# argmaxinc/WhisperKit

Hardware: NVIDIA H100
Metric: RTFx (audio-sec/s) whisper-large-v3 greedy (higher is better)
Workload: dtype bf16

## Files before the change

### whisperkit_b200/csrc/attention_wgmma.cu

```cuda
#include <stdio.h>
#include <stdlib.h>

#include "common.cuh"
#include "kernels.h"
#include "wgmma.cuh"

namespace wk {

static constexpr int kFaThreads = 384;
static constexpr int kFaBM = 128;
static constexpr int kFaBN = 128;
static constexpr int kFaD = 64;
static constexpr int kFaTile = kFaBN * kFaD * 2;
static constexpr int kFaStages = 4;
static constexpr int kFaSmem = kFaTile  + 2 * kFaStages * kFaTile  + 1024  + 256 ;

struct FaParams {
    int T, H, dm, n_kv_tiles;
    float scale_log2e;
};

__device__ __forceinline__ float fa_ex2(float x) {
    float y;
    asm("ex2.approx.ftz.f32 %0, %1;" : "=f"(y) : "f"(x));
    return y;
}

template <typename T>
__global__ void __launch_bounds__(kFaThreads, 1)
encoder_attention_wgmma_kernel(const __grid_constant__ CUtensorMap tm_qkv, T* __restrict__ out, const FaParams p) {
    extern __shared__ __align__(1024) uint8_t smem_raw[];
    uint8_t* smem = reinterpret_cast<uint8_t*>((reinterpret_cast<uintptr_t>(smem_raw) + 1023) & ~uintptr_t(1023));
    uint8_t* sQ = smem;
    uint8_t* sK = sQ + kFaTile;
    uint8_t* sV = sK + kFaStages * kFaTile;
    uint64_t* bars = reinterpret_cast<uint64_t*>(sV + kFaStages * kFaTile);
    uint64_t* q_full = bars;
    uint64_t* k_full = bars + 1;
    uint64_t* k_empty = k_full + kFaStages;
    uint64_t* v_full = k_empty + kFaStages;
    uint64_t* v_empty = v_full + kFaStages;

    const int warp = threadIdx.x >> 5, lane = threadIdx.x & 31;
    const int bh = blockIdx.y;
    const int b = bh / p.H, h = bh % p.H;
    const int q0 = blockIdx.x * kFaBM;
    const int n = p.n_kv_tiles;

    if (warp == 0 && lane == 0) {
        tma_prefetch_desc(&tm_qkv);
        mbar_init(q_full, 1);
        for (int i = 0; i < kFaStages; ++i) {
            mbar_init(&k_full[i], 1); mbar_init(&k_empty[i], 8);
            mbar_init(&v_full[i], 1); mbar_init(&v_empty[i], 8);
        }
        fence_barrier_init();
    }
    __syncthreads();

    if (warp < 4) {
        asm volatile("setmaxnreg.dec.sync.aligned.u32 40;");
        if (warp == 0 && lane == 0) {
            mbar_expect_tx(q_full, kFaTile);
            tma_load_3d(sQ, &tm_qkv, q_full, h * kFaD, q0, b);
            for (int j = 0; j < n; ++j) {
                const int st = j % kFaStages;
                const uint32_t ph = (j / kFaStages) & 1;
                mbar_wait_bounded(&k_empty[st], ph ^ 1);
                mbar_expect_tx(&k_full[st], kFaTile);
                tma_load_3d(sK + st * kFaTile, &tm_qkv, &k_full[st], p.dm + h * kFaD, j * kFaBN, b);
                mbar_wait_bounded(&v_empty[st], ph ^ 1);
                mbar_expect_tx(&v_full[st], kFaTile);
                tma_load_3d(sV + st * kFaTile, &tm_qkv, &v_full[st], 2 * p.dm + h * kFaD, j * kFaBN, b);
            }
        }
        return;
    }

    asm volatile("setmaxnreg.inc.sync.aligned.u32 232;");
    const int cw = (warp >> 2) - 1;
    const int c_lo = 2 * (lane & 3);
    const float c = p.scale_log2e;
    const uint64_t qd = wgmma_desc_sw128(smem_u32(sQ + cw * 64 * 128));
    float o[32];
#pragma unroll
    for (int i = 0; i < 32; ++i) o[i] = 0.f;
    float m_run[2] = {-INFINITY, -INFINITY}, l_run[2] = {0.f, 0.f};

    mbar_wait_bounded(q_full, 0);
    for (int j = 0; j < n; ++j) {
        const int st = j % kFaStages;
        const uint32_t ph = (j / kFaStages) & 1;
        float s[64];
        mbar_wait_bounded(&k_full[st], ph);
        const uint64_t kd = wgmma_desc_sw128(smem_u32(sK + st * kFaTile));
        wgmma_fence();
#pragma unroll
        for (int k = 0; k < kFaD / 16; ++k) Wgmma<T, 128>::ss(s, qd + (uint64_t)(2 * k), kd + (uint64_t)(2 * k), k > 0 ? 1u : 0u);
        wgmma_commit();
        wgmma_wait<0>();
        __syncwarp();
        if (lane == 0) mbar_arrive(&k_empty[st]);

        const int valid = p.T - j * kFaBN;
        if (valid < kFaBN) {
#pragma unroll
            for (int jj = 0; jj < 16; ++jj)
#pragma unroll
                for (int e = 0; e < 4; ++e)
                    if (8 * jj + c_lo + (e & 1) >= valid) s[4 * jj + e] = -INFINITY;
        }
        uint32_t pa[8][4];
#pragma unroll
        for (int hf = 0; hf < 2; ++hf) {
            float mx = m_run[hf];
#pragma unroll
            for (int jj = 0; jj < 16; ++jj) mx = fmaxf(mx, fmaxf(s[4 * jj + 2 * hf], s[4 * jj + 2 * hf + 1]));
            mx = fmaxf(mx, __shfl_xor_sync(0xffffffffu, mx, 1));
            mx = fmaxf(mx, __shfl_xor_sync(0xffffffffu, mx, 2));
            const float corr = fa_ex2((m_run[hf] - mx) * c);
            m_run[hf] = mx;
            const float nmc = -mx * c;
            float sum = 0.f;
#pragma unroll
            for (int jj = 0; jj < 16; ++jj) {
                const float e0 = fa_ex2(fmaf(s[4 * jj + 2 * hf], c, nmc));
                const float e1 = fa_ex2(fmaf(s[4 * jj + 2 * hf + 1], c, nmc));
                sum += e0 + e1;
                pa[jj >> 1][(jj & 1) * 2 + hf] = T16<T>::pack2(e0, e1);
            }
            l_run[hf] = l_run[hf] * corr + sum;
#pragma unroll
            for (int jj = 0; jj < 8; ++jj) { o[4 * jj + 2 * hf] *= corr; o[4 * jj + 2 * hf + 1] *= corr; }
        }

        mbar_wait_bounded(&v_full[st], ph);
        const uint32_t vs = smem_u32(sV + st * kFaTile);
        wgmma_fence();
#pragma unroll
        for (int kk = 0; kk < kFaBN / 16; ++kk) Wgmma<T, 64>::rs_bt(o, pa[kk], wgmma_desc_sw128(vs + kk * 2048), 1u);
        wgmma_commit();
        wgmma_wait<0>();
        __syncwarp();
        if (lane == 0) mbar_arrive(&v_empty[st]);
    }

#pragma unroll
    for (int hf = 0; hf < 2; ++hf) {
        float l = l_run[hf];
        l += __shfl_xor_sync(0xffffffffu, l, 1);
        l += __shfl_xor_sync(0xffffffffu, l, 2);
        const float inv = 1.f / l;
        const int q = q0 + cw * 64 + (warp & 3) * 16 + (lane >> 2) + 8 * hf;
        if (q >= p.T) continue;
        T* dst = out + ((long long)b * p.T + q) * p.dm + h * kFaD + c_lo;
#pragma unroll
        for (int jj = 0; jj < 8; ++jj)
            *reinterpret_cast<uint32_t*>(dst + 8 * jj) = T16<T>::pack2(o[4 * jj + 2 * hf] * inv, o[4 * jj + 2 * hf + 1] * inv);
    }
}

typedef CUresult (*PFN_encodeTiled)(CUtensorMap*, CUtensorMapDataType, cuuint32_t, void*, const cuuint64_t*, const cuuint64_t*,
                                      const cuuint32_t*, const cuuint32_t*, CUtensorMapInterleave, CUtensorMapSwizzle,
                                      CUtensorMapL2promotion, CUtensorMapFloatOOBfill);

wk_status encoder_attention_wgmma(const void* qkv, void* out, int B, int T, int n_heads, int dtype, cudaStream_t stream) {
    static PFN_encodeTiled enc = nullptr;
    if (!enc) {
        void* fp = nullptr;
        cudaDriverEntryPointQueryResult q;
        if (cudaGetDriverEntryPoint("cuTensorMapEncodeTiled", &fp, cudaEnableDefault, &q) != cudaSuccess || q != cudaDriverEntryPointSuccess) {
            set_error("cuTensorMapEncodeTiled entry point unavailable");
            return WK_ERR_CUDA;
        }
        enc = reinterpret_cast<PFN_encodeTiled>(fp);
    }
    const int dm = n_heads * 64;
    CUtensorMap tm;
    cuuint64_t gdim[3] = {(cuuint64_t)3 * dm, (cuuint64_t)T, (cuuint64_t)B};
    cuuint64_t gstr[2] = {(cuuint64_t)3 * dm * 2, (cuuint64_t)T * 3 * dm * 2};
    cuuint32_t box[3] = {64, 128, 1};
    cuuint32_t es[3] = {1, 1, 1};
    CUresult r = enc(&tm, dtype == WK_DTYPE_F16 ? CU_TENSOR_MAP_DATA_TYPE_FLOAT16 : CU_TENSOR_MAP_DATA_TYPE_BFLOAT16, 3,
                     const_cast<void*>(qkv), gdim, gstr, box, es, CU_TENSOR_MAP_INTERLEAVE_NONE, CU_TENSOR_MAP_SWIZZLE_128B,
                     CU_TENSOR_MAP_L2_PROMOTION_L2_256B, CU_TENSOR_MAP_FLOAT_OOB_FILL_NONE);
    if (r != CUDA_SUCCESS) { set_error("attention tensor map encode failed: %d", (int)r); return WK_ERR_CUDA; }
    FaParams p;
    p.T = T; p.H = n_heads; p.dm = dm;
    p.n_kv_tiles = (T + kFaBN - 1) / kFaBN;
    p.scale_log2e = 0.125f * 1.4426950408889634f;
    dim3 grid((T + kFaBM - 1) / kFaBM, B * n_heads);
    cudaError_t e = cudaSuccess;
    if (dtype == WK_DTYPE_F16) {
        static bool set = false;
        if (!set) { e = cudaFuncSetAttribute(encoder_attention_wgmma_kernel<__half>, cudaFuncAttributeMaxDynamicSharedMemorySize, kFaSmem); set = e == cudaSuccess; }
        if (e == cudaSuccess) encoder_attention_wgmma_kernel<__half><<<grid, kFaThreads, kFaSmem, stream>>>(tm, (__half*)out, p);
    } else {
        static bool set = false;
        if (!set) { e = cudaFuncSetAttribute(encoder_attention_wgmma_kernel<__nv_bfloat16>, cudaFuncAttributeMaxDynamicSharedMemorySize, kFaSmem); set = e == cudaSuccess; }
        if (e == cudaSuccess) encoder_attention_wgmma_kernel<__nv_bfloat16><<<grid, kFaThreads, kFaSmem, stream>>>(tm, (__nv_bfloat16*)out, p);
    }
    if (e != cudaSuccess) { set_error("cudaFuncSetAttribute(fa): %s", cudaGetErrorString(e)); return WK_ERR_CUDA; }
    count_launch();
    e = cudaGetLastError();
    if (e != cudaSuccess) { set_error("encoder_attention_wgmma launch: %s", cudaGetErrorString(e)); return WK_ERR_CUDA; }
    return WK_OK;
}

}
```

Measured before the change: 923.4.

## Make encoder flash attention persistent with three consumer warpgroups and QK/PV overlap

Converts the encoder attention kernel into a persistent kernel sized to the SM count. Each CTA now walks work items with a double-buffered Q slot, and the KV stage ring runs across items. Consumer warpgroups go from 2 to 3, so each item covers a 192-row query block. Inside an item, the QK wgmma for the next tile is issued before the PV wgmma of the current tile, which overlaps softmax with tensor-core work. The cost is a lower register budget per thread (160), extra Q smem, and more complex barrier logic. A second TMA load for Q rows beyond T depends on OOB fill.

```diff
diff --git a/whisperkit_b200/csrc/attention_wgmma.cu b/whisperkit_b200/csrc/attention_wgmma.cu
--- a/whisperkit_b200/csrc/attention_wgmma.cu
+++ b/whisperkit_b200/csrc/attention_wgmma.cu
@@ -7,16 +7,18 @@
 
 namespace wk {
 
-static constexpr int kFaThreads = 384;
-static constexpr int kFaBM = 128;
+static constexpr int kFaThreads = 512;
+static constexpr int kFaConsumers = 3;
+static constexpr int kFaBM = 64 * kFaConsumers;
 static constexpr int kFaBN = 128;
 static constexpr int kFaD = 64;
 static constexpr int kFaTile = kFaBN * kFaD * 2;
 static constexpr int kFaStages = 4;
-static constexpr int kFaSmem = kFaTile  + 2 * kFaStages * kFaTile  + 1024  + 256 ;
+static constexpr int kFaQSlot = 2 * kFaTile;
+static constexpr int kFaSmem = 2 * kFaQSlot  + 2 * kFaStages * kFaTile  + 1024  + 256 ;
 
 struct FaParams {
-    int T, H, dm, n_kv_tiles;
+    int T, H, dm, n_kv_tiles, n_q_blocks, n_items;
     float scale_log2e;
 };
 
@@ -24,6 +26,14 @@
     float y;
     asm("ex2.approx.ftz.f32 %0, %1;" : "=f"(y) : "f"(x));
     return y;
+}
+
+__device__ __forceinline__ void fa_wait(uint64_t* bar, uint32_t parity) {
+    if (mbar_try_wait(bar, parity)) return;
+    const unsigned long long t0 = globaltimer_ns();
+    unsigned int spins = 0;
+    while (!mbar_try_wait(bar, parity))
+        if ((++spins & 0xfffu) == 0 && globaltimer_ns() - t0 > kSpinLimitNs) __trap();
 }
 
 template <typename T>
@@ -32,76 +42,81 @@
     extern __shared__ __align__(1024) uint8_t smem_raw[];
     uint8_t* smem = reinterpret_cast<uint8_t*>((reinterpret_cast<uintptr_t>(smem_raw) + 1023) & ~uintptr_t(1023));
     uint8_t* sQ = smem;
-    uint8_t* sK = sQ + kFaTile;
+    uint8_t* sK = sQ + 2 * kFaQSlot;
     uint8_t* sV = sK + kFaStages * kFaTile;
     uint64_t* bars = reinterpret_cast<uint64_t*>(sV + kFaStages * kFaTile);
     uint64_t* q_full = bars;
-    uint64_t* k_full = bars + 1;
+    uint64_t* q_empty = bars + 2;
+    uint64_t* k_full = bars + 4;
     uint64_t* k_empty = k_full + kFaStages;
     uint64_t* v_full = k_empty + kFaStages;
     uint64_t* v_empty = v_full + kFaStages;
 
     const int warp = threadIdx.x >> 5, lane = threadIdx.x & 31;
-    const int bh = blockIdx.y;
-    const int b = bh / p.H, h = bh % p.H;
-    const int q0 = blockIdx.x * kFaBM;
     const int n = p.n_kv_tiles;
 
     if (warp == 0 && lane == 0) {
         tma_prefetch_desc(&tm_qkv);
-        mbar_init(q_full, 1);
+        for (int i = 0; i < 2; ++i) { mbar_init(&q_full[i], 1); mbar_init(&q_empty[i], 4 * kFaConsumers); }
         for (int i = 0; i < kFaStages; ++i) {
-            mbar_init(&k_full[i], 1); mbar_init(&k_empty[i], 8);
-            mbar_init(&v_full[i], 1); mbar_init(&v_empty[i], 8);
+            mbar_init(&k_full[i], 1); mbar_init(&k_empty[i], 4 * kFaConsumers);
+            mbar_init(&v_full[i], 1); mbar_init(&v_empty[i], 4 * kFaConsumers);
         }
         fence_barrier_init();
     }
     __syncthreads();
 
     if (warp < 4) {
-        asm volatile("setmaxnreg.dec.sync.aligned.u32 40;");
+        asm volatile("setmaxnreg.dec.sync.aligned.u32 32;");
         if (warp == 0 && lane == 0) {
-            mbar_expect_tx(q_full, kFaTile);
-            tma_load_3d(sQ, &tm_qkv, q_full, h * kFaD, q0, b);
-            for (int j = 0; j < n; ++j) {
-                const int st = j % kFaStages;
-                const uint32_t ph = (j / kFaStages) & 1;
-                mbar_wait_bounded(&k_empty[st], ph ^ 1);
-                mbar_expect_tx(&k_full[st], kFaTile);
-                tma_load_3d(sK + st * kFaTile, &tm_qkv, &k_full[st], p.dm + h * kFaD, j * kFaBN, b);
-                mbar_wait_bounded(&v_empty[st], ph ^ 1);
-                mbar_expect_tx(&v_full[st], kFaTile);
-                tma_load_3d(sV + st * kFaTile, &tm_qkv, &v_full[st], 2 * p.dm + h * kFaD, j * kFaBN, b);
+            uint32_t it = 0, qi = 0;
+            for (int w = blockIdx.x; w < p.n_items; w += gridDim.x, ++qi) {
+                const int bh = w / p.n_q_blocks, q0 = (w % p.n_q_blocks) * kFaBM;
+                const int b = bh / p.H, h = bh % p.H;
+                const int qs = qi & 1;
+                fa_wait(&q_empty[qs], ((qi >> 1) & 1) ^ 1);
+                mbar_expect_tx(&q_full[qs], kFaQSlot);
+                tma_load_3d(sQ + qs * kFaQSlot, &tm_qkv, &q_full[qs], h * kFaD, q0, b);
+                tma_load_3d(sQ + qs * kFaQSlot + kFaTile, &tm_qkv, &q_full[qs], h * kFaD, q0 + 128, b);
+                for (int j = 0; j < n; ++j, ++it) {
+                    const int st = it % kFaStages;
+                    const uint32_t ph = (it / kFaStages) & 1;
+                    fa_wait(&k_empty[st], ph ^ 1);
+                    mbar_expect_tx(&k_full[st], kFaTile);
+                    tma_load_3d(sK + st * kFaTile, &tm_qkv, &k_full[st], p.dm + h * kFaD, j * kFaBN, b);
+                    fa_wait(&v_empty[st], ph ^ 1);
+                    mbar_expect_tx(&v_full[st], kFaTile);
+                    tma_load_3d(sV + st * kFaTile, &tm_qkv, &v_full[st], 2 * p.dm + h * kFaD, j * kFaBN, b);
+                }
             }
         }
         return;
     }
 
-    asm volatile("setmaxnreg.inc.sync.aligned.u32 232;");
+    asm volatile("setmaxnreg.inc.sync.aligned.u32 160;");
     const int cw = (warp >> 2) - 1;
     const int c_lo = 2 * (lane & 3);
     const float c = p.scale_log2e;
-    const uint64_t qd = wgmma_desc_sw128(smem_u32(sQ + cw * 64 * 128));
-    float o[32];
-#pragma unroll
-    for (int i = 0; i < 32; ++i) o[i] = 0.f;
-    float m_run[2] = {-INFINITY, -INFINITY}, l_run[2] = {0.f, 0.f};
-
-    mbar_wait_bounded(q_full, 0);
-    for (int j = 0; j < n; ++j) {
-        const int st = j % kFaStages;
-        const uint32_t ph = (j / kFaStages) & 1;
-        float s[64];
-        mbar_wait_bounded(&k_full[st], ph);
-        const uint64_t kd = wgmma_desc_sw128(smem_u32(sK + st * kFaTile));
+    const uint32_t sK_u = smem_u32(sK), sV_u = smem_u32(sV);
+    float s[64], o[32];
+    uint32_t pa[8][4];
+    float m_run[2], l_run[2], corr[2];
+
+    auto issue_qk = [&](uint64_t qd, int st) {
+        const uint64_t kd = wgmma_desc_sw128(sK_u + st * kFaTile);
         wgmma_fence();
 #pragma unroll
         for (int k = 0; k < kFaD / 16; ++k) Wgmma<T, 128>::ss(s, qd + (uint64_t)(2 * k), kd + (uint64_t)(2 * k), k > 0 ? 1u : 0u);
         wgmma_commit();
-        wgmma_wait<0>();
-        __syncwarp();
-        if (lane == 0) mbar_arrive(&k_empty[st]);
-
+    };
+    auto issue_pv = [&](int st) {
+        const uint32_t vs = sV_u + st * kFaTile;
+        wgmma_fence();
+#pragma unroll
+        for (int kk = 0; kk < kFaBN / 16; ++kk) Wgmma<T, 64>::rs_bt(o, pa[kk], wgmma_desc_sw128(vs + kk * 2048), 1u);
+        wgmma_commit();
+    };
+    auto softmax_exp = [&](int j) {
         const int valid = p.T - j * kFaBN;
         if (valid < kFaBN) {
 #pragma unroll
@@ -110,7 +125,6 @@
                 for (int e = 0; e < 4; ++e)
                     if (8 * jj + c_lo + (e & 1) >= valid) s[4 * jj + e] = -INFINITY;
         }
-        uint32_t pa[8][4];
 #pragma unroll
         for (int hf = 0; hf < 2; ++hf) {
             float mx = m_run[hf];
@@ -118,7 +132,7 @@
             for (int jj = 0; jj < 16; ++jj) mx = fmaxf(mx, fmaxf(s[4 * jj + 2 * hf], s[4 * jj + 2 * hf + 1]));
             mx = fmaxf(mx, __shfl_xor_sync(0xffffffffu, mx, 1));
             mx = fmaxf(mx, __shfl_xor_sync(0xffffffffu, mx, 2));
-            const float corr = fa_ex2((m_run[hf] - mx) * c);
+            corr[hf] = fa_ex2((m_run[hf] - mx) * c);
             m_run[hf] = mx;
             const float nmc = -mx * c;
             float sum = 0.f;
@@ -127,36 +141,85 @@
                 const float e0 = fa_ex2(fmaf(s[4 * jj + 2 * hf], c, nmc));
                 const float e1 = fa_ex2(fmaf(s[4 * jj + 2 * hf + 1], c, nmc));
                 sum += e0 + e1;
-                pa[jj >> 1][(jj & 1) * 2 + hf] = T16<T>::pack2(e0, e1);
+                s[4 * jj + 2 * hf] = e0; s[4 * jj + 2 * hf + 1] = e1;
             }
-            l_run[hf] = l_run[hf] * corr + sum;
-#pragma unroll
-            for (int jj = 0; jj < 8; ++jj) { o[4 * jj + 2 * hf] *= corr; o[4 * jj + 2 * hf + 1] *= corr; }
-        }
-
-        mbar_wait_bounded(&v_full[st], ph);
-        const uint32_t vs = smem_u32(sV + st * kFaTile);
-        wgmma_fence();
-#pragma unroll
-        for (int kk = 0; kk < kFaBN / 16; ++kk) Wgmma<T, 64>::rs_bt(o, pa[kk], wgmma_desc_sw128(vs + kk * 2048), 1u);
-        wgmma_commit();
+            l_run[hf] = l_run[hf] * corr[hf] + sum;
+        }
+#pragma unroll
+        for (int i = 0; i < 64; ++i) asm volatile("" : "+f"(s[i])::"memory");
+    };
+    auto softmax_pack = [&]() {
+#pragma unroll
+        for (int hf = 0; hf < 2; ++hf) {
+#pragma unroll
+            for (int jj = 0; jj < 16; ++jj)
+                pa[jj >> 1][(jj & 1) * 2 + hf] = T16<T>::pack2(s[4 * jj + 2 * hf], s[4 * jj + 2 * hf + 1]);
+#pragma unroll
+            for (int jj = 0; jj < 8; ++jj) { o[4 * jj + 2 * hf] *= corr[hf]; o[4 * jj + 2 * hf + 1] *= corr[hf]; }
+        }
+    };
+
+    uint32_t it = 0, qi = 0;
+    for (int w = blockIdx.x; w < p.n_items; w += gridDim.x, ++qi) {
+        const int bh = w / p.n_q_blocks, q0 = (w % p.n_q_blocks) * kFaBM;
+        const int b = bh / p.H, h = bh % p.H;
+        const int qs = qi & 1;
+        const uint64_t qd = wgmma_desc_sw128(smem_u32(sQ + qs * kFaQSlot + cw * 64 * 128));
+#pragma unroll
+        for (int i = 0; i < 32; ++i) o[i] = 0.f;
+        m_run[0] = m_run[1] = -INFINITY;
+        l_run[0] = l_run[1] = 0.f;
+
+        fa_wait(&q_full[qs], (qi >> 1) & 1);
+        fa_wait(&k_full[it % kFaStages], (it / kFaStages) & 1);
+        issue_qk(qd, it % kFaStages);
         wgmma_wait<0>();
         __syncwarp();
-        if (lane == 0) mbar_arrive(&v_empty[st]);
-    }
-
-#pragma unroll
-    for (int hf = 0; hf < 2; ++hf) {
-        float l = l_run[hf];
-        l += __shfl_xor_sync(0xffffffffu, l, 1);
-        l += __shfl_xor_sync(0xffffffffu, l, 2);
-        const float inv = 1.f / l;
-        const int q = q0 + cw * 64 + (warp & 3) * 16 + (lane >> 2) + 8 * hf;
-        if (q >= p.T) continue;
-        T* dst = out + ((long long)b * p.T + q) * p.dm + h * kFaD + c_lo;
-#pragma unroll
-        for (int jj = 0; jj < 8; ++jj)
-            *reinterpret_cast<uint32_t*>(dst + 8 * jj) = T16<T>::pack2(o[4 * jj + 2 * hf] * inv, o[4 * jj + 2 * hf + 1] * inv);
+        if (lane == 0) {
+            mbar_arrive(&k_empty[it % kFaStages]);
+            if (n == 1) mbar_arrive(&q_empty[qs]);
+        }
+        softmax_exp(0);
+        softmax_pack();
+
+        for (int j = 0; j + 1 < n; ++j, ++it) {
+            const int st = it % kFaStages, st1 = (it + 1) % kFaStages;
+            fa_wait(&k_full[st1], ((it + 1) / kFaStages) & 1);
+            issue_qk(qd, st1);
+            fa_wait(&v_full[st], (it / kFaStages) & 1);
+            issue_pv(st);
+            wgmma_wait<1>();
+            softmax_exp(j + 1);
+            __syncwarp();
+            if (lane == 0) {
+                mbar_arrive(&k_empty[st1]);
+                if (j + 2 == n) mbar_arrive(&q_empty[qs]);
+            }
+            wgmma_wait<0>();
+            __syncwarp();
+            if (lane == 0) mbar_arrive(&v_empty[st]);
+            softmax_pack();
+        }
+        fa_wait(&v_full[it % kFaStages], (it / kFaStages) & 1);
+        issue_pv(it % kFaStages);
+        wgmma_wait<0>();
+        __syncwarp();
+        if (lane == 0) mbar_arrive(&v_empty[it % kFaStages]);
+        ++it;
+
+#pragma unroll
+        for (int hf = 0; hf < 2; ++hf) {
+            float l = l_run[hf];
+            l += __shfl_xor_sync(0xffffffffu, l, 1);
+            l += __shfl_xor_sync(0xffffffffu, l, 2);
+            const float inv = 1.f / l;
+            const int q = q0 + cw * 64 + (warp & 3) * 16 + (lane >> 2) + 8 * hf;
+            if (q >= p.T) continue;
+            T* dst = out + ((long long)b * p.T + q) * p.dm + h * kFaD + c_lo;
+#pragma unroll
+            for (int jj = 0; jj < 8; ++jj)
+                *reinterpret_cast<uint32_t*>(dst + 8 * jj) = T16<T>::pack2(o[4 * jj + 2 * hf] * inv, o[4 * jj + 2 * hf + 1] * inv);
+        }
     }
 }
 
@@ -188,9 +251,14 @@
     FaParams p;
     p.T = T; p.H = n_heads; p.dm = dm;
     p.n_kv_tiles = (T + kFaBN - 1) / kFaBN;
+    p.n_q_blocks = (T + kFaBM - 1) / kFaBM;
+    p.n_items = p.n_q_blocks * B * n_heads;
     p.scale_log2e = 0.125f * 1.4426950408889634f;
-    dim3 grid((T + kFaBM - 1) / kFaBM, B * n_heads);
-    cudaError_t e = cudaSuccess;
+    int dev = 0, num_sms = 0;
+    cudaError_t e = cudaGetDevice(&dev);
+    if (e == cudaSuccess) e = cudaDeviceGetAttribute(&num_sms, cudaDevAttrMultiProcessorCount, dev);
+    if (e != cudaSuccess) { set_error("encoder_attention_wgmma: SM count: %s", cudaGetErrorString(e)); return WK_ERR_CUDA; }
+    const dim3 grid(p.n_items < num_sms ? p.n_items : num_sms);
     if (dtype == WK_DTYPE_F16) {
         static bool set = false;
         if (!set) { e = cudaFuncSetAttribute(encoder_attention_wgmma_kernel<__half>, cudaFuncAttributeMaxDynamicSharedMemorySize, kFaSmem); set = e == cudaSuccess; }
```

New measurement: 932.9, median of 6. 1.01x the previous value.
